# Berkeley-Speech-Group/sylber

Hardware: AMD Instinct MI355X
Metric: audio-sec/s encoded (sylber_base, 16 kHz, batched 10 s clips) (higher is better)
Workload: dtype bf16; 1 GPU; Segmenter forward (conv frontend + HuBERT-9L encoder + boundary detection + segment mean-pool), batch 32 x 10 s 16 kHz random waveforms per GPU, random-init sylber_base weights (BASELINE.json configs[1]); global_batch=32, frames_per_clip=499, parallelism=utterance-sharded x1, shards resident per rank, no data-path collective, rccl_ranks=1

## Files before the change

### include/sylber_hip.h

```cpp
#ifndef SYLBER_HIP_H
#define SYLBER_HIP_H

#include <stdint.h>

#ifdef __cplusplus
extern "C" {
#endif

#define SYLBER_MAX_LAYERS 12
#define SYLBER_HIDDEN 768
#define SYLBER_CONV_DIM 512

typedef struct sylber_ctx* sylber_t;

enum { SYLBER_BF16 = 0, SYLBER_FP32 = 1, SYLBER_FP8 = 2, SYLBER_FP16 = 3, SYLBER_MIXED16 = 4, SYLBER_SPLIT16 = 5 };

typedef struct {
    const float* q_w; const float* q_b;
    const float* k_w; const float* k_b;
    const float* v_w; const float* v_b;
    const float* o_w; const float* o_b;
    const float* ln1_w; const float* ln1_b;
    const float* ff1_w; const float* ff1_b;
    const float* ff2_w; const float* ff2_b;
// ... 276 lines not shown
int sylber_condition_units(sylber_mlp_t m, const float* c1_dev, int32_t K1, const float* c2_dev, int32_t K2, const int32_t* units_dev,
                           const int32_t* spans_dev, const int32_t* nunits_dev, const int32_t* frames_dev, int32_t B, int32_t T, int32_t S,
                           float* cond_dev, float* workspace_dev, void* stream);
int64_t sylber_condition_packed_workspace_floats(sylber_mlp_t m, int32_t B, int32_t S);
int sylber_condition_packed(sylber_mlp_t m, const float* hidden_dev, const int32_t* offsets_host, const int32_t* frames_host, int32_t B,
                            const int64_t* seg_dev, const int32_t* nseg_dev, const float* feat_dev, int32_t K, int32_t S, float norm_thr,
                            float* avg_hidden_dev, float* cond_dev, float* workspace_dev, void* stream);
int sylber_condition_units_packed(sylber_mlp_t m, const float* c1_dev, int32_t K1, const float* c2_dev, int32_t K2, const int32_t* units_dev,
                                  const int32_t* spans_dev, const int32_t* nunits_dev, const int32_t* frames_host, int32_t B, int32_t S,
                                  float* cond_dev, float* workspace_dev, void* stream);
int sylber_expand_units(const float* feats_dev, const int32_t* durations_dev, int32_t B, int32_t S, int32_t D, int32_t T, float* out_dev,
                        int32_t* workspace_dev, void* stream);

enum { SYLBER_OPT_GEMM_TILE = 1, SYLBER_OPT_ATTN_QUERIES_PER_WAVE = 2, SYLBER_OPT_GEMM_PERSISTENT = 3, SYLBER_OPT_FUSE_OUTPROJ_LN = 4,
       SYLBER_OPT_CONV0_VALU = 5, SYLBER_OPT_RESLN_PREFETCH = 6, SYLBER_OPT_FP8_ATTENTION = 7, SYLBER_OPT_GEMM_TAIL = 8, SYLBER_OPT_SEGMENT = 9, SYLBER_OPT_FP16_AUDIT = 10, SYLBER_OPT_GEMM_H192 = 11, SYLBER_OPT_GEMM_MODEL = 12, SYLBER_OPT_GEMM_MFMA16 = 13,
       SYLBER_OPT_PER_UTTERANCE = 14 };
int sylber_set_option(sylber_t h, int32_t key, int32_t value);
int sylber_get_fp16_audit(sylber_t h, const char** names, uint32_t* saturated, float* max_abs, int32_t cap);

int sylber_condition_features(sylber_mlp_t m, const float* features_dev, int32_t rows, float* cond_dev, float* workspace_dev,
                              void* stream);

enum { SYLBER_TAP_CONV0 = -1, SYLBER_TAP_PROJ = -2, SYLBER_TAP_POSCONV = -3 };
enum { SYLBER_LTAP_QKV = 0, SYLBER_LTAP_CTX = 1, SYLBER_LTAP_ATTN_SUM = 2, SYLBER_LTAP_LN1 = 3, SYLBER_LTAP_FFN1 = 4, SYLBER_LTAP_FFN2_SUM = 5 };
#define SYLBER_TAP_LAYER(l, k) (-(8 * ((l) + 1) + (k)))
#define SYLBER_TAP_CONV(i) (-(1024 + (i)))
int sylber_set_stop_stage(sylber_t h, int32_t stage);
int sylber_set_profiling(sylber_t h, int32_t enable);
int sylber_get_profile(sylber_t h, const char** names, float* ms, int32_t cap);
int sylber_set_graph_mode(sylber_t h, int32_t enable);
int64_t sylber_workspace_bytes(sylber_t h);
// ... 53 lines not shown
```

### sylber_amd/_lib.py

```python
from __future__ import annotations

import ctypes
import os
from ctypes import POINTER, c_char_p, c_float, c_int, c_int32, c_int64, c_void_p

_HERE = os.path.dirname(os.path.abspath(__file__))
LIB_PATH = os.path.join(_HERE, "libsylber_hip.so")
_DEV_LIB = False
MAX_LAYERS = 12

c_float_p = POINTER(c_float)


class SylberLayerWeights(ctypes.Structure):
    _fields_ = [(n, c_float_p) for n in (
        "q_w", "q_b", "k_w", "k_b", "v_w", "v_b", "o_w", "o_b", "ln1_w", "ln1_b",
        "ff1_w", "ff1_b", "ff2_w", "ff2_b", "ln2_w", "ln2_b")]


class SylberMlpHidden(ctypes.Structure):
    _fields_ = [(n, c_float_p) for n in ("lin_w", "lin_b", "ff1_w", "ff1_b", "ff2_w", "ff2_b", "ln_w", "ln_b")]


class SylberMlpWeights(ctypes.Structure):
# ... 220 lines not shown
    "sylber_cfm_tap_floats_packed": (c_int64, [c_void_p, c_int32, POINTER(c_int32), c_int32]),
    "sylber_debug_segment_scalars": (c_int, [c_void_p, c_void_p, c_int64, c_void_p, c_void_p, c_void_p, c_void_p, c_void_p, c_void_p, c_int64,
                                             c_void_p, c_void_p]),
}
CFM_TAP_CONDX, CFM_TAP_GB, CFM_TAP_XE, CFM_TAP_X0 = 1, 2, 3, 4
(CFM_BTAP_H_ATTN, CFM_BTAP_QKV, CFM_BTAP_Q, CFM_BTAP_K, CFM_BTAP_VT, CFM_BTAP_QKVF, CFM_BTAP_CTX, CFM_BTAP_X_ATTN, CFM_BTAP_H_FF, CFM_BTAP_FF,
 CFM_BTAP_G, CFM_BTAP_X_FF) = range(12)


def CFM_TAP(block: int, k: int) -> int:
    return 16 * (int(block) + 1) + int(k)
OPT_GEMM_TILE, OPT_ATTN_QUERIES_PER_WAVE, OPT_GEMM_PERSISTENT = 1, 2, 3
OPT_FUSE_OUTPROJ_LN, OPT_CONV0_VALU = 4, 5
OPT_FP8_ATTENTION, OPT_SEGMENT, OPT_PER_UTTERANCE = 7, 9, 14
OPT_GEMM_MODEL, OPT_GEMM_MFMA16 = 12, 13
TAP_CONV0, TAP_PROJ, TAP_POSCONV = -1, -2, -3
LTAP_QKV, LTAP_CTX, LTAP_ATTN_SUM, LTAP_LN1, LTAP_FFN1, LTAP_FFN2_SUM = 0, 1, 2, 3, 4, 5
LTAP_WIDTH = {LTAP_QKV: 2304, LTAP_CTX: 768, LTAP_ATTN_SUM: 768, LTAP_LN1: 768, LTAP_FFN1: 3072, LTAP_FFN2_SUM: 768}


def ltap_width(k: int, precision: str = "bf16", fp8_attention: bool = True) -> int:
    w = LTAP_WIDTH.get(int(k), 768)
    if precision != "fp8" or k in (LTAP_ATTN_SUM, LTAP_FFN2_SUM) or (k == LTAP_QKV and not fp8_attention):
        return w
    return 2 * w


def TAP_LAYER(l: int, k: int) -> int:
    return -(8 * (int(l) + 1) + int(k))

# ... 41 lines not shown
```

### sylber_amd/csrc/api.hip

```cpp
#include "ctx.h"

static thread_local char g_err[512] = "";
void syl_set_error(const char* what, const char* detail) { snprintf(g_err, sizeof(g_err), "%s: %s", what, detail); }
extern "C" const char* sylber_last_error(void) { return g_err; }

struct Packer {
    std::vector<char> host;
    size_t add(size_t bytes) { size_t off = (host.size() + 255) & ~(size_t)255; host.resize(off + bytes); return off; }
    size_t add_f32(const float* src, size_t n) { size_t o = add(n * 4); memcpy(host.data() + o, src, n * 4); return o; }
    int fmt = FMT_BF16;
    size_t add_bf16(const float* src, size_t n) {
        if (fmt == FMT_SPLIT) {
            size_t o = add(n * 4);
            bf16_t* d = (bf16_t*)(host.data() + o);
            for (size_t i = 0; i < n; ++i) { d[i] = f2h_host(src[i]); d[n + i] = f2h_host(src[i] - h2f_host(d[i])); }
            return o;
        }
        size_t o = add(n * 2);
        bf16_t* d = (bf16_t*)(host.data() + o);
        if (fmt == FMT_F16) for (size_t i = 0; i < n; ++i) d[i] = f2h_host(src[i]);
        else for (size_t i = 0; i < n; ++i) d[i] = f2bf(src[i]);
        return o;
    }
};
// ... 39 lines not shown
            for (int n = 0; n < 48; ++n)
                for (int cc = 0; cc < 48; ++cc)
                    for (int t = 0; t < 128; ++t)
                        tmp[(((size_t)g * 128 + t) * 64 + n) * 56 + cc] = w->pos_w[(((size_t)g * 48 + n) * 48 + cc) * 128 + t];
        if (!f32) o_posw = P.add_bf16(tmp.data(), tmp.size());
        else {
            std::vector<float> t32((size_t)16 * 128 * 64 * 52, 0.f);
            for (int g = 0; g < 16; ++g)
                for (int n = 0; n < 48; ++n)
                    for (int cc = 0; cc < 48; ++cc)
                        for (int t = 0; t < 128; ++t)
                            t32[(((size_t)g * 128 + t) * 64 + n) * 52 + cc] = w->pos_w[(((size_t)g * 48 + n) * 48 + cc) * 128 + t];
            o_posw = P.add_f32(t32.data(), t32.size());
        }
    }
    size_t o_posb = P.add_f32(w->pos_b, 768);
    size_t o_elw = P.add_f32(w->enc_ln_w, 768), o_elb = P.add_f32(w->enc_ln_b, 768);
    struct LOff { size_t wqkv, bqkv, wo, bo, l1w, l1b, w1, b1, w2, b2, l2w, l2b; } lo[SYLBER_MAX_LAYERS];
    for (int l = 0; l < w->num_layers; ++l) {
        const SylberLayerWeights& lw = w->layers[l];
        std::vector<float> qkv((size_t)2304 * 768), bq(2304);
        memcpy(qkv.data(), lw.q_w, 768 * 768 * 4);
        memcpy(qkv.data() + 768 * 768, lw.k_w, 768 * 768 * 4);
        memcpy(qkv.data() + 2 * 768 * 768, lw.v_w, 768 * 768 * 4);
        memcpy(bq.data(), lw.q_b, 768 * 4); memcpy(bq.data() + 768, lw.k_b, 768 * 4); memcpy(bq.data() + 1536, lw.v_b, 768 * 4);
        lo[l].wqkv = f32 ? P.add_f32(qkv.data(), qkv.size()) : P.add_bf16(qkv.data(), qkv.size()); lo[l].bqkv = P.add_f32(bq.data(), 2304);
        lo[l].wo = f32 ? P.add_f32(lw.o_w, 768 * 768) : P.add_bf16(lw.o_w, 768 * 768); lo[l].bo = P.add_f32(lw.o_b, 768);
        lo[l].l1w = P.add_f32(lw.ln1_w, 768); lo[l].l1b = P.add_f32(lw.ln1_b, 768);
        lo[l].w1 = f32 ? P.add_f32(lw.ff1_w, (size_t)3072 * 768) : P.add_bf16(lw.ff1_w, (size_t)3072 * 768); lo[l].b1 = P.add_f32(lw.ff1_b, 3072);
        lo[l].w2 = f32 ? P.add_f32(lw.ff2_w, (size_t)768 * 3072) : P.add_bf16(lw.ff2_w, (size_t)768 * 3072); lo[l].b2 = P.add_f32(lw.ff2_b, 768);
        lo[l].l2w = P.add_f32(lw.ln2_w, 768); lo[l].l2b = P.add_f32(lw.ln2_b, 768);
    }
    c->wbytes = P.host.size();
    if (hipMalloc((void**)&c->wbase, c->wbytes) != hipSuccess) { delete c; syl_set_error("sylber_create", "hipMalloc(weights) failed"); return 1; }
    if (hipMemcpy(c->wbase, P.host.data(), c->wbytes, hipMemcpyHostToDevice) != hipSuccess) {
        hipFree(c->wbase); delete c; syl_set_error("sylber_create", "weight upload failed"); return 1;
    }
    char* b = c->wbase;
    c->conv0_w = (float*)(b + o_conv0); c->gn_w = (float*)(b + o_gnw); c->gn_b = (float*)(b + o_gnb);
    c->conv_w[0] = nullptr;
    for (int i = 1; i < 7; ++i) { c->conv_w[i] = (bf16_t*)(b + o_conv[i]); c->conv_w32[i] = (float*)(b + o_conv[i]); }
    c->fp_w32 = (float*)(b + o_fpw); c->pos_w32 = (float*)(b + o_posw);
    c->fp_ln_w = (float*)(b + o_fplw); c->fp_ln_b = (float*)(b + o_fplb);
    c->fp_w = (bf16_t*)(b + o_fpw); c->fp_b = (float*)(b + o_fpb);
    c->pos_w = (bf16_t*)(b + o_posw); c->pos_b = (float*)(b + o_posb);
    c->enc_ln_w = (float*)(b + o_elw); c->enc_ln_b = (float*)(b + o_elb);
    for (int l = 0; l < w->num_layers; ++l) {
        LayerDev& d = c->L[l];
        d.wqkv = (bf16_t*)(b + lo[l].wqkv); d.bqkv = (float*)(b + lo[l].bqkv);
        d.wo = (bf16_t*)(b + lo[l].wo); d.bo = (float*)(b + lo[l].bo);
        d.ln1w = (float*)(b + lo[l].l1w); d.ln1b = (float*)(b + lo[l].l1b);
        d.w1 = (bf16_t*)(b + lo[l].w1); d.b1 = (float*)(b + lo[l].b1);
        d.w2 = (bf16_t*)(b + lo[l].w2); d.b2 = (float*)(b + lo[l].b2);
        d.ln2w = (float*)(b + lo[l].l2w); d.ln2b = (float*)(b + lo[l].l2b);
        c->L32[l].wqkv = (float*)(b + lo[l].wqkv); c->L32[l].wo = (float*)(b + lo[l].wo);
        c->L32[l].w1 = (float*)(b + lo[l].w1); c->L32[l].w2 = (float*)(b + lo[l].w2);
    }
    if (precision == SYLBER_FP8) {
        const size_t per_layer = (size_t)3072 * 768 + (size_t)3072 * 24 + (size_t)768 * 3072 + (size_t)768 * 96 +
                                 (size_t)2304 * 768 + (size_t)2304 * 24 + (size_t)768 * 768 + (size_t)768 * 24;
// ... 78 lines not shown
            GUARD_DEVICE(c->device);
            c->opt_audit16 = value > 0 ? 1 : 0;
            if (c->opt_audit16) {
                if (!c->audit_dev) HIP_TRY(hipMalloc((void**)&c->audit_dev, AUDIT_STAGES * 2 * sizeof(unsigned)));
                HIP_TRY(hipDeviceSynchronize());
                HIP_TRY(hipMemset(c->audit_dev, 0, AUDIT_STAGES * 2 * sizeof(unsigned)));
            }
            break;
        }
        case SYLBER_OPT_SEGMENT: c->opt_segment = value < 0 ? -1 : 0; break;
        case SYLBER_OPT_GEMM_MODEL: c->opt_gemm_model = value == 5 ? 5 : (value == 2 ? 2 : (value == 6 ? 6 : 0)); break;
        case SYLBER_OPT_GEMM_H192: c->opt_gemm_h192 = value < 0 ? -1 : 0; break;
        case SYLBER_OPT_GEMM_MFMA16: c->opt_gemm_mfma16 = value < 0 ? -1 : 0; break;
        case SYLBER_OPT_GEMM_TAIL: c->opt_gemm_tail = value < 0 ? -1 : (value > 0 ? value + 1 : 0); break;
        case SYLBER_OPT_PER_UTTERANCE: c->opt_per_utt = value == 1 ? 1 : 0; break;
        default: syl_set_error("sylber_set_option", "unknown option key"); return 1;
    }
    if (c->graph_mode) graphs_clear(c);
    return 0;
}
extern "C" int sylber_set_profiling(sylber_t c, int32_t enable) {
    if (!c) return 1;
    const char* nm[1]; float ms[1];
    sylber_get_profile(c, nm, ms, 0);
    c->prof_names.clear(); c->prof_ms.clear();
    c->profiling = enable;
    return 0;
}
extern "C" int64_t sylber_workspace_bytes(sylber_t c) { return c ? (int64_t)(c->ws_bytes + c->seg_scratch_floats * 4 + c->wbytes + c->f8bytes) : 0; }

// ... 96 lines not shown
```

### sylber_amd/csrc/ctx.h

```cpp
#pragma once
#include <stdio.h>
#include <stdlib.h>
#include <string.h>

#include <string>
#include <vector>

#include "../../include/sylber_hip.h"
#include "../../include/sylber_hip_dev.h"
#include "kernels.h"

struct DeviceGuard {
    int prev = -1; bool ok = true;
    explicit DeviceGuard(int dev) {
        if (hipGetDevice(&prev) != hipSuccess) prev = -1;
        if (prev != dev) ok = hipSetDevice(dev) == hipSuccess;
    }
    ~DeviceGuard() { int cur = -1; if (prev >= 0 && hipGetDevice(&cur) == hipSuccess && cur != prev) (void)hipSetDevice(prev); }
};
#define GUARD_DEVICE(dev)                                                                             \
    DeviceGuard _dg(dev);                                                                             \
    if (!_dg.ok) { syl_set_error("hipSetDevice", "cannot select the handle's device"); return 1; }

static const int CK[7] = {10, 3, 3, 3, 3, 2, 2};
// ... 9 lines not shown

struct ProfEntry { std::string name; hipEvent_t e0, e1; };
struct GraphEntry { int B, Lmax, stop_stage; const void* in; void* out; hipGraphExec_t exec; unsigned long long stamp; };

enum { AUD_CONV0 = 0, AUD_CONV6 = 6, AUD_LN512 = 7, AUD_XPAD = 8, AUD_LN = 9, AUD_Q = 10, AUD_K = 11, AUD_V = 12, AUD_CTX = 13, AUD_FFN1 = 14, AUDIT_STAGES = 15 };

struct sylber_ctx {
    int device = 0, precision = 0, num_layers = 9;
    int fmt = FMT_BF16;
    int fmt_conv = FMT_BF16;
    char* wbase = nullptr; size_t wbytes = 0;
    char* f8base = nullptr; size_t f8bytes = 0;
    float *conv0_w, *gn_w, *gn_b, *fp_ln_w, *fp_ln_b, *fp_b, *pos_b, *enc_ln_w, *enc_ln_b;
    bf16_t* conv_w[7];
    bf16_t *fp_w, *pos_w;
    LayerDev L[SYLBER_MAX_LAYERS];
    float* conv_w32[7]; float *fp_w32, *pos_w32;
    struct { float *wqkv, *wo, *w1, *w2; } L32[SYLBER_MAX_LAYERS];
    char* ws = nullptr; size_t ws_bytes = 0;
    int ws_B = 0, ws_Lmax = 0;
    float* seg_scratch = nullptr; size_t seg_scratch_floats = 0;
    int stop_stage = 0;
    const float* dbg_ss = nullptr; int dbg_ss_B = 0;
    int opt_gemm_cfg = 0, opt_attn_qw = 0, opt_gemm_persist = 0;
    int opt_fuse_ln = 0;
    int opt_conv0_valu = 0;
    int opt_audit16 = 0;
    unsigned* audit_dev = nullptr;
    int opt_segment = 0;
    int opt_gemm_model = 0;
    int opt_gemm_mfma16 = 0;
    int opt_gemm_h192 = 0;
    int opt_gemm_tail = 0;
    int opt_attn8 = 0;
    int opt_resln_pre = 0;
    int opt_per_utt = 0;
    bool graph_mode = false;
    std::vector<GraphEntry> graphs; unsigned long long graph_clock = 0;
    int profiling = 0;
    std::vector<ProfEntry> prof;
    std::vector<hipEvent_t> ev_pool;
    std::vector<std::string> prof_names; std::vector<float> prof_ms;
};

void graphs_clear(sylber_ctx* c);

struct ProfScope {
    sylber_ctx* c; hipStream_t s; bool on;
    ProfScope(sylber_ctx* c_, hipStream_t s_, const char* name) : c(c_), s(s_), on(c_->profiling != 0) {
        if (!on) return;
// ... 14 lines not shown
```

### sylber_amd/csrc/forward.hip

```cpp
#include "ctx.h"

extern "C" int32_t sylber_num_frames(int32_t n) {
    for (int i = 0; i < 7; ++i) n = (n - CK[i]) / CS[i] + 1;
    return n;
}

static int frames_needed(int Lmax) {
    int n = Lmax, tp = 0;
    for (int i = 0; i < 7; ++i) {
        n = (n - CK[i]) / CS[i] + 1;
        const int f = 1 << (6 - i);
        const int need = (n + f - 1) / f;
        tp = need > tp ? need : tp;
    }
    return tp;
}
static int padded_frames(int Lmax) { return (frames_needed(Lmax) + 31) & ~31; }
extern "C" int32_t sylber_padded_frames(int32_t n_samples) { return n_samples < 400 ? 0 : padded_frames(n_samples); }

#define SYL_SLOT_ALIGN 64
extern "C" int sylber_packed_layout(const int32_t* samples_host, int32_t B, int32_t* offsets, int32_t* frames) {
    if (!samples_host || !offsets || !frames || B < 1) { syl_set_error("sylber_packed_layout", "need B >= 1 and non-null arrays"); return 1; }
    const long long cap = (long long)INT32_MAX / SYL_SLOT_SAMPLES;
    long long off = 0;
// ... 337 lines not shown
        LnArgs a = {};
        a.in = feats; a.in_bf16 = 1; a.ld_in = 512; a.gamma = c->fp_ln_w; a.beta = c->fp_ln_b;
        a.out_bf16 = w.ln512; a.ld_bf16 = 512; a.M = M; a.D = 512; a.fmt = c->fmt; a.fmt_in = c->fmt_conv;
        a.in_lo = feats_lo; a.out_lo = p.lo_ln512;
        RUN("ln512", launch_layernorm(a, s));
        GemmArgs g = linear(w.ln512, p.lo_ln512, c->fp_w, c->fp_b, 768, 512);
        g.out0 = w.xf32; g.ld0 = 768; g.out1 = w.xpad; g.Tp = p.Tp; g.T = p.T; g.valid = w.valid; g.xpad_rows = p.Tp + 128; g.out_lo = p.lo_xpad;
        RUN("gemm_proj", launch_gemm_bf16(EPI_PROJ, g, s));
        if (pk) RUN("zero_slot_tails", launch_zero_slot_tails(w.xf32, w.xpad, pk->slot, pk->frames, pk->nclip, pk->tail_max, s));
        AUDIT(aud_e, AUD_LN512, w.ln512, M, 512, 512);
        AUDIT(aud_e, AUD_XPAD, w.xpad, (long)B * (p.Tp + 128), 768, 768);
        return 0;
    }

    int posconv() {
        if (pk) RUN("posconv", launch_posconv_packed(w.xpad, c->pos_w, c->pos_b, w.xf32, w.pre, pk->nclip, pk->slot_max, pk->slot, pk->frames, s, c->fmt));
        else RUN("posconv", launch_posconv(w.xpad, c->pos_w, c->pos_b, w.xf32, w.pre, B, p.Tp, split ? 2 : 1, s, c->fmt, p.lo_xpad, (long)16 * 128 * 64 * 56));
        return 0;
    }

    int layernorm(const float* gam, const float* bet, bool last) {
        LnArgs a = {};
        a.in = w.pre; a.in_bf16 = 0; a.ld_in = 768; a.gamma = gam; a.beta = bet; a.M = M; a.D = 768; a.fmt = c->fmt; a.fmt_in = c->fmt;
        if (last) { a.out_f32 = hidden_dev; a.ld_f32 = 768; a.Tp = p.Tp; a.T = p.T; }
        else if (f8) { a.out_fp8 = w8.h; a.ld_fp8 = 768; a.out_scale = w8.hs; a.scale_rows = w8.Mp; a.out_stats = w.stats; }
        else { a.out_bf16 = w.h; a.ld_bf16 = 768; a.out_stats = w.stats; a.out_lo = p.lo_hbf; }
        if (launch_layernorm(a, s)) return 1;
        AUDIT(aud_e && !last && !f8, AUD_LN, w.h, M, 768, 768);
        return 0;
    }

    int tap_rows16(const bf16_t* buf, long lo, int W) {
// ... 298 lines not shown
    const bool f32 = c->precision == SYLBER_FP32;
    const Plan p = f32 ? make_plan_f32(B, Lmax) : make_plan(B, Lmax, c->precision == SYLBER_SPLIT16 ? 2 : 1);
    if (begin_call(c, p, {{p.o_valid, valid.data(), B}, {p.o_rows, c->opt_per_utt ? rows0.data() : nullptr, B}}, s)) return 1;
    c->dbg_ss = (const float*)(c->ws + p.o_ss); c->dbg_ss_B = B;
    if (f32) return ForwardF32(c, p, wav_dev, hidden_dev, s).run();
    if (!c->graph_mode || c->profiling || c->opt_audit16 || s == nullptr || c->stop_stage < 0) return Forward(c, p, wav_dev, hidden_dev, s, nullptr).run();
    return forward_graph(c, p, wav_dev, hidden_dev, s);
}

extern "C" int sylber_forward_packed(sylber_t c, const float* wav_dev, const int32_t* samples_host, int32_t B, float* hidden_dev, void* stream) {
    if (!c || !wav_dev || !samples_host || !hidden_dev) { syl_set_error("sylber_forward_packed", "null argument"); return 1; }
    if (c->precision != SYLBER_BF16 && c->precision != SYLBER_FP16) {
        syl_set_error("sylber_forward_packed", "packed batches run in the bf16 and fp16 precisions only"); return 1;
    }
    if (c->graph_mode) { syl_set_error("sylber_forward_packed", "not available in graph mode (sylber_set_graph_mode)"); return 1; }
    if (c->stop_stage != 0 || c->opt_conv0_valu != 0 || c->opt_attn_qw != 0) {
        syl_set_error("sylber_forward_packed", "not available with a stop stage, SYLBER_OPT_CONV0_VALU or SYLBER_OPT_ATTN_QUERIES_PER_WAVE"); return 1;
    }
    std::vector<int32_t> off(B > 0 ? B + 1 : 1), fr(B > 0 ? B : 1);
    if (sylber_packed_layout(samples_host, B, off.data(), fr.data())) return 1;
    const int Ptot = off[B];
    std::vector<int32_t> tab(3 * (size_t)B + 2), rows0(B);
    int slot_max = 0, tail_max = 0, nmax = 0;
    tab[2 * B + 1] = 0;
    for (int b = 0; b < B; ++b) {
        const int sl = off[b + 1] - off[b];
        slot_max = sl > slot_max ? sl : slot_max;
        tail_max = sl - fr[b] > tail_max ? sl - fr[b] : tail_max;
        rows0[b] = (samples_host[b] - CK[0]) / CS[0] + 1;
        nmax = samples_host[b] > nmax ? samples_host[b] : nmax;
        tab[B + 1 + b] = fr[b];
        tab[2 * B + 2 + b] = tab[2 * B + 1 + b] + (fr[b] + 127) / 128;
// ... 44 lines not shown
```

### sylber_amd/csrc/kernels.h

```cpp
#pragma once
#include "common.h"

enum GemmAct { ACT_NONE = 0, ACT_GELU_FAST = 1, ACT_GELU_ERF = 2, ACT_GELU_ERF7 = 3 };
enum GemmEpi {
    EPI_BF16 = 0,
    EPI_F32 = 1,
    EPI_F32_RES = 2,
    EPI_QK = 3,
    EPI_PROJ = 4,
    EPI_MXFP8 = 7,
    EPI_QK8 = 8,
    EPI_F32_RESLN = 6,
};

struct GemmArgs {
    const bf16_t* X; long ldx;
    const bf16_t* W;
    int M, N, K;
    int M_store;
    const float* bias;
    int act;
    void* out0; long ld0;
    void* out1; void* out2;
    const float* res; long ldres;
// ... 59 lines not shown
};
int launch_gemm_f32(const GemmArgsF32& a, hipStream_t s);
int launch_km_normalize(const float* x, float* y, int n, int D, hipStream_t s);
int launch_km_sqnorm(const float* c, float* out, int K, int D, hipStream_t s);

int launch_conv0_stats(const float* wav, int B, int Lmax, int L0, double* partials, int nchunk, hipStream_t s, const int* rows = nullptr,
                       const int* slot = nullptr);
int launch_conv0_finalize(const double* partials, int nchunk, const float* w0, const float* gn_w, const float* gn_b,
                          int B, int L0, float* scale_shift, hipStream_t s, const int* rows = nullptr);
int launch_conv0_gn_gelu(const float* wav, int B, int Lmax, int L0, int R0, const float* w0,
                         const float* scale_shift, void* out, int out_f32, hipStream_t s, int fmt = 0, long out_lo = 0, int valu16 = 0);
int launch_conv0_packed(const float* wav, int B, int total_samples, int slot_max, const int* rows, const int* slot, const float* w0,
                        const float* scale_shift, bf16_t* out, int fmt, hipStream_t s);
int launch_zero_slot_tails(float* x, bf16_t* xpad, const int* slot, const int* frames, int B, int tail_max, hipStream_t s);
int launch_posconv_packed(const bf16_t* xpad, const bf16_t* wpk, const float* bias, const float* x_f32, float* out, int B, int slot_max,
                          const int* slot, const int* frames, hipStream_t s, int fmt);
int launch_attention_packed(const bf16_t* q, const bf16_t* k, const bf16_t* vt, const int* pk, int nclip, int total_qb, bf16_t* ctx,
                            int Ptot, hipStream_t s, int fmt);

struct LnArgs {
    const void* in; int in_bf16; long ld_in;
    int fmt;
    int fmt_in;
    const float* res; long ld_res;
    const float* gamma; const float* beta;
    float* out_f32; long ld_f32;
    bf16_t* out_bf16; long ld_bf16;
    uint8_t* out_fp8; long ld_fp8;
    uint8_t* out_scale; long scale_rows;
    float* out_stats;
    int M, D;
    int Tp, T;
    long in_lo, out_lo;
};
int launch_layernorm(const LnArgs& a, hipStream_t s);

int launch_attention(const bf16_t* q, const bf16_t* k, const bf16_t* vt, const int* valid, bf16_t* ctx, int B, int T,
                     int Tp, int Tpv, int qw, hipStream_t s, int fmt = 0, long lo_qk = 0, long lo_vt = 0, long lo_ctx = 0);
int launch_attention_f8(const uint8_t* q8, const uint8_t* qs, const uint8_t* k8, const uint8_t* ks, const uint8_t* v8, const uint8_t* vs,
                        const int* valid, void* ctx, uint8_t* ctx_scale, long scale_rows, int B, int T, int Tp, int Tpv, hipStream_t s);
int launch_attention_f8out(const bf16_t* q, const bf16_t* k, const bf16_t* vt, const int* valid, uint8_t* ctx8, uint8_t* ctx_scale,
                           long scale_rows, int B, int T, int Tp, int Tpv, int qw, hipStream_t s);
int launch_attention_f32(const float* q, const float* k, const float* v, const int* valid, float* ctx, int B, int T,
                         int Tp, hipStream_t s);

int launch_posconv(const bf16_t* xpad, const bf16_t* wpk, const float* bias, const float* x_f32, float* out, int B,
                   int Tp, int act, hipStream_t s, int fmt = 0, long x_lo = 0, long w_lo = 0);
int launch_posconv_f32(const float* xpad, const float* w, const float* bias, const float* x_f32, float* out, int B,
                       int Tp, hipStream_t s);

int launch_segment(const float* hidden, int B, int T, int D, float norm_thr, float merge_thr, int64_t* seg, int* nseg,
                   float* feat, float* scratch, hipStream_t s, int mode = 0, const int* frames = nullptr, const int* row0 = nullptr);
size_t segment_scratch_floats(int B, int T, int D);

int launch_upload_ints(int* dst, const int32_t* vals_host, int n, int add, hipStream_t s);
int launch_f32_to_bf16(const float* in, bf16_t* out, size_t n, hipStream_t s);
int launch_f32_to_split16(const float* in, bf16_t* out, long lo_off, size_t n, hipStream_t s);
int launch_bf16_to_f32_rows(const bf16_t* in, long ld_in, float* out, int B, int Tp, int T, int D, hipStream_t s, int fmt = 0, long in_lo = 0);
enum { MXTAP_ROWS = 0, MXTAP_HEADS = 1, MXTAP_VT = 2 };
int launch_mxfp8_to_f32_rows(const uint8_t* data, const uint8_t* scale, int layout, long pitch, float* out, long ld_out, int val_col, int exp_col,
                             int B, int Tp, int T, int W, hipStream_t s);
int launch_tap_qkv(const bf16_t* q, const bf16_t* k, const bf16_t* vt, float* out, int B, int T, int Tp, int Tpv, hipStream_t s, int fmt, long lo_qk, long lo_vt);
// ... 1 lines not shown
```

### sylber_amd/csrc/posconv.hip

```cpp
#include "kernels.h"
#include "lds_dma.h"

#define PC_BM 256
#define PC_XROW 112
#define PC_XWIN (384 * PC_XROW)
#define PC_SLAB (64 * 112)
#define PC_TAPS_PER_STEP 2
#define PC_STEP (PC_TAPS_PER_STEP * PC_SLAB)
#define PC_LDS (PC_XWIN + 2 * PC_STEP)

template <int ACT, int FMT>
__global__ __launch_bounds__(512, 4) void posconv_bf16_kernel(const bf16_t* __restrict__ xpad, const bf16_t* __restrict__ wpk,
                                                              const float* __restrict__ bias, const float* __restrict__ x_f32,
                                                              float* __restrict__ out, int Tp, long x_lo, long w_lo,
                                                              const int* __restrict__ slot, const int* __restrict__ frames) {
    extern __shared__ __attribute__((aligned(256))) char smem[];
    char* xwin = smem;
    char* wring = smem + PC_XWIN;
    const int tid = threadIdx.x, wave = tid >> 6, lane = tid & 63;
    const int ql = lane & 31, h = lane >> 5;
    const int t0 = blockIdx.x * PC_BM, g = blockIdx.y, b = blockIdx.z;
    const int rows_per_b = Tp + 128;
    int s0 = 0, Tb = 0, Tpb = Tp;
    if (slot) {
// ... 74 lines not shown
                const int nl = 32 * nf + 8 * gg + 4 * h;
                if (nl >= SYL_POSC) continue;
                const int n = g * SYL_POSC + nl;
                const float4 bb = *(const float4*)(bias + n);
                const float4 rr = *(const float4*)(x_f32 + m * SYL_HIDDEN + n);
                float v0 = acc[nf][4 * gg + 0] + bb.x, v1 = acc[nf][4 * gg + 1] + bb.y;
                float v2 = acc[nf][4 * gg + 2] + bb.z, v3 = acc[nf][4 * gg + 3] + bb.w;
                if constexpr (ACT == 2 && FMT == FMT_SPLIT) { v0 = gelu_erf7(v0); v1 = gelu_erf7(v1); v2 = gelu_erf7(v2); v3 = gelu_erf7(v3); }
                else if constexpr (ACT == 2) { v0 = gelu_erf(v0); v1 = gelu_erf(v1); v2 = gelu_erf(v2); v3 = gelu_erf(v3); }
                else { v0 = gelu_fast(v0); v1 = gelu_fast(v1); v2 = gelu_fast(v2); v3 = gelu_fast(v3); }
                *(float4*)(out + m * SYL_HIDDEN + n) = make_float4(rr.x + v0, rr.y + v1, rr.z + v2, rr.w + v3);
            }
    }
}

static int posconv_attrs() {
    static PerDeviceOnce attr_once;
    if (attr_once.need()) {
        HIP_TRY(hipFuncSetAttribute((const void*)posconv_bf16_kernel<1, FMT_BF16>, hipFuncAttributeMaxDynamicSharedMemorySize, PC_LDS));
        HIP_TRY(hipFuncSetAttribute((const void*)posconv_bf16_kernel<2, FMT_BF16>, hipFuncAttributeMaxDynamicSharedMemorySize, PC_LDS));
        HIP_TRY(hipFuncSetAttribute((const void*)posconv_bf16_kernel<1, FMT_F16>, hipFuncAttributeMaxDynamicSharedMemorySize, PC_LDS));
        HIP_TRY(hipFuncSetAttribute((const void*)posconv_bf16_kernel<2, FMT_SPLIT>, hipFuncAttributeMaxDynamicSharedMemorySize, PC_LDS));
    }
    return 0;
}

int launch_posconv(const bf16_t* xpad, const bf16_t* wpk, const float* bias, const float* x_f32, float* out, int B, int Tp,
                   int act, hipStream_t s, int fmt, long x_lo, long w_lo) {
    dim3 grid((Tp + PC_BM - 1) / PC_BM, SYL_POSG, B);
    if (posconv_attrs()) return 1;
    if (fmt == FMT_SPLIT) {
        hipLaunchKernelGGL((posconv_bf16_kernel<2, FMT_SPLIT>), grid, dim3(512), PC_LDS, s, xpad, wpk, bias, x_f32, out, Tp, x_lo, w_lo, nullptr, nullptr);
        HIP_TRY(hipGetLastError());
        return 0;
    }
    if (fmt == FMT_F16 && act == 2) { syl_set_error("launch_posconv", "the erf GELU (act 2) has no fp16 instantiation"); return 1; }
    if (fmt == FMT_F16) hipLaunchKernelGGL((posconv_bf16_kernel<1, FMT_F16>), grid, dim3(512), PC_LDS, s, xpad, wpk, bias, x_f32, out, Tp, 0L, 0L, nullptr, nullptr);
    else if (act == 2) hipLaunchKernelGGL((posconv_bf16_kernel<2, FMT_BF16>), grid, dim3(512), PC_LDS, s, xpad, wpk, bias, x_f32, out, Tp, 0L, 0L, nullptr, nullptr);
    else hipLaunchKernelGGL((posconv_bf16_kernel<1, FMT_BF16>), grid, dim3(512), PC_LDS, s, xpad, wpk, bias, x_f32, out, Tp, 0L, 0L, nullptr, nullptr);
    HIP_TRY(hipGetLastError());
    return 0;
}

int launch_posconv_packed(const bf16_t* xpad, const bf16_t* wpk, const float* bias, const float* x_f32, float* out, int B, int slot_max,
                          const int* slot, const int* frames, hipStream_t s, int fmt) {
    if (fmt != FMT_BF16 && fmt != FMT_F16) { syl_set_error("launch_posconv_packed", "bf16 / fp16 only"); return 1; }
    if (posconv_attrs()) return 1;
    dim3 grid((slot_max + PC_BM - 1) / PC_BM, SYL_POSG, B);
    if (fmt == FMT_F16) hipLaunchKernelGGL((posconv_bf16_kernel<1, FMT_F16>), grid, dim3(512), PC_LDS, s, xpad, wpk, bias, x_f32, out, 0, 0L, 0L, slot, frames);
    else hipLaunchKernelGGL((posconv_bf16_kernel<1, FMT_BF16>), grid, dim3(512), PC_LDS, s, xpad, wpk, bias, x_f32, out, 0, 0L, 0L, slot, frames);
    HIP_TRY(hipGetLastError());
    return 0;
}
```

### sylber_amd/segmenter.py

```python
from __future__ import annotations

import ctypes
import math
import os
import collections
import threading
import time
import weakref
from pathlib import Path
from typing import Dict, List, Optional, Sequence, Union

import numpy as np
import torch

from . import _lib
from .ingest import ingest_file
from .weights import (NUM_LAYERS, expected_shapes, fold_pos_conv_weight, normalize_keys, synthetic_state_dict)

FRAME_RATE = 50
SLOT_SAMPLES = 320
PACKED_PRECISIONS = ("bf16", "fp16")


def _ptr(t: torch.Tensor):
# ... 322 lines not shown
    def set_graph_mode(self, enable: bool = True) -> None:
        _lib.check(self.lib.sylber_set_graph_mode(self.handle, 1 if enable else 0), "sylber_set_graph_mode")
        self._graph_stream = torch.cuda.Stream(device=self.device) if enable else None

    def _check_packed(self, what: str) -> None:
        if self.precision not in PACKED_PRECISIONS:
            raise ValueError("%s: packed batches run in precision %s only (this encoder: %r)" % (what, " / ".join(map(repr, PACKED_PRECISIONS)),
                                                                                                   self.precision))
        if getattr(self, "_graph_stream", None) is not None:
            raise ValueError("%s: packed batches do not run in graph mode (set_graph_mode(False))" % what)
        if self._opts.get(_lib.OPT_SEGMENT, 0) < 0:
            raise ValueError("%s: packed boundary detection needs the wide segmenter (SYLBER_OPT_SEGMENT = 0, not -1)" % what)
        if (self._opts.get(_lib.OPT_ATTN_QUERIES_PER_WAVE, 0) in (32, 64) or self._opts.get(_lib.OPT_CONV0_VALU, 0) > 0):
            raise ValueError("%s: packed batches need SYLBER_OPT_ATTN_QUERIES_PER_WAVE and SYLBER_OPT_CONV0_VALU at their defaults" % what)

    def forward_packed_raw(self, wav: torch.Tensor, lengths: Sequence[int], out: Optional[torch.Tensor] = None, layout=None) -> torch.Tensor:
        self._check_packed("forward_packed")
        n = [int(x) for x in lengths]
        offsets, _ = packed_layout(n) if layout is None else layout
        P = int(offsets[-1])
        assert wav.is_cuda and wav.dtype == torch.float32 and wav.is_contiguous() and wav.numel() == SLOT_SAMPLES * P
        if out is None:
            out = torch.empty(P, 768, dtype=torch.float32, device=wav.device)
        assert out.is_contiguous() and out.numel() >= P * 768
        with torch.cuda.device(wav.device):
            st = self.lib.sylber_forward_packed(self.handle, ctypes.c_void_p(wav.data_ptr()), (ctypes.c_int32 * len(n))(*n), len(n),
                                                ctypes.c_void_p(out.data_ptr()), _stream_ptr(wav.device))
        _lib.check(st, "sylber_forward_packed")
        return out

    def forward_packed(self, wavs: Sequence[torch.Tensor]):
        self._check_packed("forward_packed")
        rows = [torch.as_tensor(w).reshape(-1) for w in wavs]
        lengths = [int(r.numel()) for r in rows]
        offsets, frames = packed_layout(lengths)
        wav = torch.zeros(SLOT_SAMPLES * int(offsets[-1]), dtype=torch.float32, device=self.device)
        for i, r in enumerate(rows):
            a = SLOT_SAMPLES * int(offsets[i])
            wav[a:a + lengths[i]] = r.to(self.device, torch.float32)
        return self.forward_packed_raw(wav, lengths), offsets, frames

    def segment_packed(self, hidden: torch.Tensor, lengths: Sequence[int], norm_threshold: float, merge_threshold: float,
                       with_features: bool = True, out=None, layout=None):
        self._check_packed("segment_packed")
        n = [int(x) for x in lengths]
        offsets, frames = packed_layout(n) if layout is None else layout
        assert hidden.is_cuda and hidden.dtype == torch.float32 and hidden.is_contiguous() and hidden.numel() >= int(offsets[-1]) * 768
        B, K, D = len(n), int(frames.max()), 768
        if out is not None:
            seg, nseg, feats = out
        else:
            seg = torch.empty(B, K, 2, dtype=torch.int64, device=hidden.device)
            nseg = torch.empty(B, dtype=torch.int32, device=hidden.device)
            feats = torch.empty(B, K, D, dtype=torch.float32, device=hidden.device) if with_features else None
        with torch.cuda.device(hidden.device):
# ... 555 lines not shown
```

Baseline: 67520 audio-sec/s.

## Add 16x16x32 MFMA positional-conv kernel with prepacked weights and LDS ring

Adds a new grouped positional-convolution kernel built on 16x16x32 bf16/fp16 MFMA instructions. It uses a host-repacked weight layout that pairs taps, stages the input window in LDS, and streams weights through a 2- or 3-slot LDS ring filled by async global-to-LDS loads. Bias, GELU and the residual add are fused into its epilogue. The kernel is selected by a new option whose default value routes both the padded and packed paths to it. The change also allows a posconv stop stage for packed batches, and it adds an extra weight copy in device memory.

```diff
diff --git a/include/sylber_hip.h b/include/sylber_hip.h
--- a/include/sylber_hip.h
+++ b/include/sylber_hip.h
@@ -314,7 +314,7 @@
 
 enum { SYLBER_OPT_GEMM_TILE = 1, SYLBER_OPT_ATTN_QUERIES_PER_WAVE = 2, SYLBER_OPT_GEMM_PERSISTENT = 3, SYLBER_OPT_FUSE_OUTPROJ_LN = 4,
        SYLBER_OPT_CONV0_VALU = 5, SYLBER_OPT_RESLN_PREFETCH = 6, SYLBER_OPT_FP8_ATTENTION = 7, SYLBER_OPT_GEMM_TAIL = 8, SYLBER_OPT_SEGMENT = 9, SYLBER_OPT_FP16_AUDIT = 10, SYLBER_OPT_GEMM_H192 = 11, SYLBER_OPT_GEMM_MODEL = 12, SYLBER_OPT_GEMM_MFMA16 = 13,
-       SYLBER_OPT_PER_UTTERANCE = 14 };
+       SYLBER_OPT_PER_UTTERANCE = 14, SYLBER_OPT_POSCONV = 15 };
 int sylber_set_option(sylber_t h, int32_t key, int32_t value);
 int sylber_get_fp16_audit(sylber_t h, const char** names, uint32_t* saturated, float* max_abs, int32_t cap);
 
diff --git a/sylber_amd/_lib.py b/sylber_amd/_lib.py
--- a/sylber_amd/_lib.py
+++ b/sylber_amd/_lib.py
@@ -258,6 +258,7 @@
 OPT_FUSE_OUTPROJ_LN, OPT_CONV0_VALU = 4, 5
 OPT_FP8_ATTENTION, OPT_SEGMENT, OPT_PER_UTTERANCE = 7, 9, 14
 OPT_GEMM_MODEL, OPT_GEMM_MFMA16 = 12, 13
+OPT_POSCONV = 15
 TAP_CONV0, TAP_PROJ, TAP_POSCONV = -1, -2, -3
 LTAP_QKV, LTAP_CTX, LTAP_ATTN_SUM, LTAP_LN1, LTAP_FFN1, LTAP_FFN2_SUM = 0, 1, 2, 3, 4, 5
 LTAP_WIDTH = {LTAP_QKV: 2304, LTAP_CTX: 768, LTAP_ATTN_SUM: 768, LTAP_LN1: 768, LTAP_FFN1: 3072, LTAP_FFN2_SUM: 768}
diff --git a/sylber_amd/csrc/api.hip b/sylber_amd/csrc/api.hip
--- a/sylber_amd/csrc/api.hip
+++ b/sylber_amd/csrc/api.hip
@@ -77,6 +77,17 @@
             o_posw = P.add_f32(t32.data(), t32.size());
         }
     }
+    size_t o_posw16 = 0;
+    const bool pos16 = !f32 && c->fmt != FMT_SPLIT;
+    if (pos16) {
+        std::vector<float> tmp((size_t)16 * 64 * 48 * 96);
+        for (int g = 0; g < 16; ++g)
+            for (int n = 0; n < 48; ++n)
+                for (int cc = 0; cc < 48; ++cc)
+                    for (int t = 0; t < 128; ++t)
+                        tmp[(((size_t)g * 64 + t / 2) * 48 + n) * 96 + (t & 1) * 48 + cc] = w->pos_w[(((size_t)g * 48 + n) * 48 + cc) * 128 + t];
+        o_posw16 = P.add_bf16(tmp.data(), tmp.size());
+    }
     size_t o_posb = P.add_f32(w->pos_b, 768);
     size_t o_elw = P.add_f32(w->enc_ln_w, 768), o_elb = P.add_f32(w->enc_ln_b, 768);
     struct LOff { size_t wqkv, bqkv, wo, bo, l1w, l1b, w1, b1, w2, b2, l2w, l2b; } lo[SYLBER_MAX_LAYERS];
@@ -107,6 +118,7 @@
     c->fp_ln_w = (float*)(b + o_fplw); c->fp_ln_b = (float*)(b + o_fplb);
     c->fp_w = (bf16_t*)(b + o_fpw); c->fp_b = (float*)(b + o_fpb);
     c->pos_w = (bf16_t*)(b + o_posw); c->pos_b = (float*)(b + o_posb);
+    c->pos_w16 = pos16 ? (bf16_t*)(b + o_posw16) : nullptr;
     c->enc_ln_w = (float*)(b + o_elw); c->enc_ln_b = (float*)(b + o_elb);
     for (int l = 0; l < w->num_layers; ++l) {
         LayerDev& d = c->L[l];
@@ -215,6 +227,7 @@
         case SYLBER_OPT_GEMM_MFMA16: c->opt_gemm_mfma16 = value < 0 ? -1 : 0; break;
         case SYLBER_OPT_GEMM_TAIL: c->opt_gemm_tail = value < 0 ? -1 : (value > 0 ? value + 1 : 0); break;
         case SYLBER_OPT_PER_UTTERANCE: c->opt_per_utt = value == 1 ? 1 : 0; break;
+        case SYLBER_OPT_POSCONV: c->opt_posconv = value < 0 ? -1 : (value <= 2 ? value : 0); break;
         default: syl_set_error("sylber_set_option", "unknown option key"); return 1;
     }
     if (c->graph_mode) graphs_clear(c);
diff --git a/sylber_amd/csrc/ctx.h b/sylber_amd/csrc/ctx.h
--- a/sylber_amd/csrc/ctx.h
+++ b/sylber_amd/csrc/ctx.h
@@ -47,6 +47,7 @@
     float *conv0_w, *gn_w, *gn_b, *fp_ln_w, *fp_ln_b, *fp_b, *pos_b, *enc_ln_w, *enc_ln_b;
     bf16_t* conv_w[7];
     bf16_t *fp_w, *pos_w;
+    bf16_t* pos_w16 = nullptr;
     LayerDev L[SYLBER_MAX_LAYERS];
     float* conv_w32[7]; float *fp_w32, *pos_w32;
     struct { float *wqkv, *wo, *w1, *w2; } L32[SYLBER_MAX_LAYERS];
@@ -67,6 +68,7 @@
     int opt_gemm_tail = 0;
     int opt_attn8 = 0;
     int opt_resln_pre = 0;
+    int opt_posconv = 0;
     int opt_per_utt = 0;
     bool graph_mode = false;
     std::vector<GraphEntry> graphs; unsigned long long graph_clock = 0;
diff --git a/sylber_amd/csrc/forward.hip b/sylber_amd/csrc/forward.hip
--- a/sylber_amd/csrc/forward.hip
+++ b/sylber_amd/csrc/forward.hip
@@ -375,8 +375,8 @@
     }
 
     int posconv() {
-        if (pk) RUN("posconv", launch_posconv_packed(w.xpad, c->pos_w, c->pos_b, w.xf32, w.pre, pk->nclip, pk->slot_max, pk->slot, pk->frames, s, c->fmt));
-        else RUN("posconv", launch_posconv(w.xpad, c->pos_w, c->pos_b, w.xf32, w.pre, B, p.Tp, split ? 2 : 1, s, c->fmt, p.lo_xpad, (long)16 * 128 * 64 * 56));
+        if (pk) RUN("posconv", launch_posconv_packed(w.xpad, c->pos_w, c->pos_b, w.xf32, w.pre, pk->nclip, pk->slot_max, pk->slot, pk->frames, s, c->fmt, c->pos_w16, c->opt_posconv));
+        else RUN("posconv", launch_posconv(w.xpad, c->pos_w, c->pos_b, w.xf32, w.pre, B, p.Tp, split ? 2 : 1, s, c->fmt, p.lo_xpad, (long)16 * 128 * 64 * 56, c->pos_w16, c->opt_posconv));
         return 0;
     }
 
@@ -705,8 +705,8 @@
         syl_set_error("sylber_forward_packed", "packed batches run in the bf16 and fp16 precisions only"); return 1;
     }
     if (c->graph_mode) { syl_set_error("sylber_forward_packed", "not available in graph mode (sylber_set_graph_mode)"); return 1; }
-    if (c->stop_stage != 0 || c->opt_conv0_valu != 0 || c->opt_attn_qw != 0) {
-        syl_set_error("sylber_forward_packed", "not available with a stop stage, SYLBER_OPT_CONV0_VALU or SYLBER_OPT_ATTN_QUERIES_PER_WAVE"); return 1;
+    if ((c->stop_stage != 0 && c->stop_stage != SYLBER_TAP_POSCONV) || c->opt_conv0_valu != 0 || c->opt_attn_qw != 0) {
+        syl_set_error("sylber_forward_packed", "not available with a stop stage other than SYLBER_TAP_POSCONV, SYLBER_OPT_CONV0_VALU or SYLBER_OPT_ATTN_QUERIES_PER_WAVE"); return 1;
     }
     std::vector<int32_t> off(B > 0 ? B + 1 : 1), fr(B > 0 ? B : 1);
     if (sylber_packed_layout(samples_host, B, off.data(), fr.data())) return 1;
diff --git a/sylber_amd/csrc/kernels.h b/sylber_amd/csrc/kernels.h
--- a/sylber_amd/csrc/kernels.h
+++ b/sylber_amd/csrc/kernels.h
@@ -97,7 +97,7 @@
                         const float* scale_shift, bf16_t* out, int fmt, hipStream_t s);
 int launch_zero_slot_tails(float* x, bf16_t* xpad, const int* slot, const int* frames, int B, int tail_max, hipStream_t s);
 int launch_posconv_packed(const bf16_t* xpad, const bf16_t* wpk, const float* bias, const float* x_f32, float* out, int B, int slot_max,
-                          const int* slot, const int* frames, hipStream_t s, int fmt);
+                          const int* slot, const int* frames, hipStream_t s, int fmt, const bf16_t* w16 = nullptr, int variant = -1);
 int launch_attention_packed(const bf16_t* q, const bf16_t* k, const bf16_t* vt, const int* pk, int nclip, int total_qb, bf16_t* ctx,
                             int Ptot, hipStream_t s, int fmt);
 
@@ -128,7 +128,7 @@
                          int Tp, hipStream_t s);
 
 int launch_posconv(const bf16_t* xpad, const bf16_t* wpk, const float* bias, const float* x_f32, float* out, int B,
-                   int Tp, int act, hipStream_t s, int fmt = 0, long x_lo = 0, long w_lo = 0);
+                   int Tp, int act, hipStream_t s, int fmt = 0, long x_lo = 0, long w_lo = 0, const bf16_t* w16 = nullptr, int variant = -1);
 int launch_posconv_f32(const float* xpad, const float* w, const float* bias, const float* x_f32, float* out, int B,
                        int Tp, hipStream_t s);
 
diff --git a/sylber_amd/csrc/posconv.hip b/sylber_amd/csrc/posconv.hip
--- a/sylber_amd/csrc/posconv.hip
+++ b/sylber_amd/csrc/posconv.hip
@@ -112,9 +112,157 @@
     }
 }
 
+#define P16_BM 256
+#define P16_XROW 96
+#define P16_XWIN (384 * P16_XROW)
+#define P16_WROW 224
+#define P16_GSTEP (SYL_POSC * 96 * 2)
+#define P16_PIECES 11
+#define P16_SLOT (P16_PIECES * 1024)
+#define P16_LDS(NS) (P16_XWIN + (NS) * P16_SLOT)
+
+template <int FMT> struct Mfma16 {
+    static __device__ __forceinline__ f32x4_t mfma(bf16x8_t a, bf16x8_t b, f32x4_t c) { return __builtin_amdgcn_mfma_f32_16x16x32_bf16(a, b, c, 0, 0, 0); }
+};
+template <> struct Mfma16<FMT_F16> {
+    static __device__ __forceinline__ f32x4_t mfma(bf16x8_t a, bf16x8_t b, f32x4_t c) {
+        return __builtin_amdgcn_mfma_f32_16x16x32_f16(__builtin_bit_cast(f16x8_t, a), __builtin_bit_cast(f16x8_t, b), c, 0, 0, 0);
+    }
+};
+
+template <int FMT, int NS>
+__global__ __launch_bounds__(256, 2) void posconv16_kernel(const bf16_t* __restrict__ xpad, const bf16_t* __restrict__ w16,
+                                                           const float* __restrict__ bias, const float* __restrict__ x_f32,
+                                                           float* __restrict__ out, int Tp, const int* __restrict__ slot,
+                                                           const int* __restrict__ frames) {
+    extern __shared__ __attribute__((aligned(256))) char smem[];
+    char* xwin = smem;
+    char* wring = smem + P16_XWIN;
+    const int tid = threadIdx.x, wave = __builtin_amdgcn_readfirstlane(tid >> 6), lane = tid & 63;
+    const int fr = lane & 15, kq = lane >> 4;
+    const int t0 = blockIdx.x * P16_BM, g = blockIdx.y, b = blockIdx.z;
+    const int rows_per_b = Tp + 128;
+    int s0 = 0, Tb = 0, Tpb = Tp;
+    if (slot) {
+        s0 = slot[b]; Tb = frames[b]; Tpb = slot[b + 1] - s0;
+        if (t0 >= Tpb) return;
+    }
+
+    {
+        const bf16_t* xb = xpad + (slot ? (size_t)s0 : (size_t)b * rows_per_b) * SYL_HIDDEN + g * SYL_POSC;
+        uint4 v[9];
+#pragma unroll
+        for (int i = 0; i < 9; ++i) {
+            const int idx = tid + 256 * i;
+            const int r = idx / 6, ch = idx - r * 6;
+            if (slot) {
+                const int f = t0 + r - 64;
+                v[i] = (f >= 0 && f < Tb) ? *(const uint4*)(xb + (size_t)(f + 64) * SYL_HIDDEN + ch * 8) : make_uint4(0u, 0u, 0u, 0u);
+            } else {
+                int row = t0 + r; row = row < rows_per_b ? row : rows_per_b - 1;
+                v[i] = *(const uint4*)(xb + (size_t)row * SYL_HIDDEN + ch * 8);
+            }
+        }
+#pragma unroll
+        for (int i = 0; i < 9; ++i) *(uint4*)(xwin + (tid + 256 * i) * 16) = v[i];
+    }
+    const __amdgpu_buffer_rsrc_t rwg = make_rsrc((const char*)w16 + (size_t)g * (SYL_POSK / 2) * P16_GSTEP);
+    int voff[3];
+#pragma unroll
+    for (int i = 0; i < 3; ++i) {
+        const int ci = (wave + 4 * i) * 64 + lane;
+        int row = ci / 14, cc = ci - row * 14;
+        row = row < SYL_POSC ? row : SYL_POSC - 1; cc = cc < 12 ? cc : 11;
+        voff[i] = row * 192 + cc * 16;
+    }
+    auto stage = [&](int step, int buf) {
+        char* dst = wring + buf * P16_SLOT;
+#pragma unroll
+        for (int i = 0; i < 3; ++i) {
+            const int piece = wave + 4 * i;
+            if (piece < P16_PIECES) glds16b(rwg, voff[i], step * P16_GSTEP, dst + piece * 1024);
+        }
+    };
+
+    f32x4_t acc[4][3];
+#pragma unroll
+    for (int fb = 0; fb < 4; ++fb)
+#pragma unroll
+        for (int nb = 0; nb < 3; ++nb) acc[fb][nb] = f32x4_t{0.f, 0.f, 0.f, 0.f};
+
+    const int xfrag = (wave * 64 + fr) * P16_XROW + kq * 16;
+    const int wfrag = fr * P16_WROW + kq * 16;
+    constexpr int nsteps = SYL_POSK / 2;
+#pragma unroll
+    for (int i = 0; i < NS - 1; ++i) stage(i, i);
+    bf16x8_t wf[2][3], xf[2][4];
+    auto load_w = [&](bf16x8_t (&d)[3], const char* p) {
+#pragma unroll
+        for (int nb = 0; nb < 3; ++nb) d[nb] = *(const bf16x8_t*)(p + nb * 16 * P16_WROW);
+    };
+    auto load_x = [&](bf16x8_t (&d)[4], const char* p) {
+#pragma unroll
+        for (int fb = 0; fb < 4; ++fb) d[fb] = *(const bf16x8_t*)(p + fb * 16 * P16_XROW);
+    };
+    static_assert(nsteps % 2 == 0, "two steps per trip");
+#pragma unroll 1
+    for (int st2 = 0; st2 < nsteps; st2 += 2) {
+#pragma unroll
+        for (int hh = 0; hh < 2; ++hh) {
+            const int st = st2 + hh;
+            if (NS == 3 && st + 1 < nsteps) {
+                if (wave == 3) wait_vmcnt<2>(); else wait_vmcnt<3>();
+            } else wait_vmcnt<0>();
+            __syncthreads();
+            if (st + NS - 1 < nsteps) stage(st + NS - 1, (st + NS - 1) % NS);
+            const char* wb = wring + (st % NS) * P16_SLOT + wfrag;
+            const char* xs = xwin + xfrag + st * (2 * P16_XROW);
+            if (st == 0) load_x(xf[0], xs);
+            load_w(wf[hh], wb);
+#pragma unroll
+            for (int sl = 0; sl < 3; ++sl) {
+                const int cur = (3 * hh + sl) & 1, nxt = cur ^ 1;
+                if (sl < 2) { load_w(wf[nxt], wb + (sl + 1) * 64); load_x(xf[nxt], xs + (sl + 1) * 64); }
+                else if (st + 1 < nsteps) load_x(xf[nxt], xs + 2 * P16_XROW);
+#pragma unroll
+                for (int fb = 0; fb < 4; ++fb)
+#pragma unroll
+                    for (int nb = 0; nb < 3; ++nb) acc[fb][nb] = Mfma16<FMT>::mfma(wf[cur][nb], xf[cur][fb], acc[fb][nb]);
+            }
+        }
+    }
+#pragma unroll
+    for (int fb = 0; fb < 4; ++fb) {
+        const int t = t0 + wave * 64 + fb * 16 + fr;
+        if (t >= Tpb) continue;
+        const size_t m = slot ? (size_t)s0 + t : (size_t)b * Tp + t;
+#pragma unroll
+        for (int nb = 0; nb < 3; ++nb) {
+            const int n = g * SYL_POSC + nb * 16 + kq * 4;
+            const float4 bb = *(const float4*)(bias + n);
+            const float4 rr = *(const float4*)(x_f32 + m * SYL_HIDDEN + n);
+            const float v0 = gelu_fast(acc[fb][nb][0] + bb.x), v1 = gelu_fast(acc[fb][nb][1] + bb.y);
+            const float v2 = gelu_fast(acc[fb][nb][2] + bb.z), v3 = gelu_fast(acc[fb][nb][3] + bb.w);
+            *(float4*)(out + m * SYL_HIDDEN + n) = make_float4(rr.x + v0, rr.y + v1, rr.z + v2, rr.w + v3);
+        }
+    }
+}
+
+#define P16_LDS_ONE_PER_CU (96 * 1024)
+template <int FMT>
+static void posconv16_launch(int variant, dim3 grid, hipStream_t s, const bf16_t* xpad, const bf16_t* w16, const float* bias, const float* x_f32,
+                             float* out, int Tp, const int* slot, const int* frames) {
+    if (variant == 1) hipLaunchKernelGGL((posconv16_kernel<FMT, 3>), grid, dim3(256), P16_LDS(3), s, xpad, w16, bias, x_f32, out, Tp, slot, frames);
+    else hipLaunchKernelGGL((posconv16_kernel<FMT, 2>), grid, dim3(256), variant == 2 ? P16_LDS_ONE_PER_CU : P16_LDS(2), s, xpad, w16, bias, x_f32, out, Tp, slot, frames);
+}
+
 static int posconv_attrs() {
     static PerDeviceOnce attr_once;
     if (attr_once.need()) {
+        HIP_TRY(hipFuncSetAttribute((const void*)posconv16_kernel<FMT_BF16, 2>, hipFuncAttributeMaxDynamicSharedMemorySize, P16_LDS_ONE_PER_CU));
+        HIP_TRY(hipFuncSetAttribute((const void*)posconv16_kernel<FMT_F16, 2>, hipFuncAttributeMaxDynamicSharedMemorySize, P16_LDS_ONE_PER_CU));
+        HIP_TRY(hipFuncSetAttribute((const void*)posconv16_kernel<FMT_BF16, 3>, hipFuncAttributeMaxDynamicSharedMemorySize, P16_LDS(3)));
+        HIP_TRY(hipFuncSetAttribute((const void*)posconv16_kernel<FMT_F16, 3>, hipFuncAttributeMaxDynamicSharedMemorySize, P16_LDS(3)));
         HIP_TRY(hipFuncSetAttribute((const void*)posconv_bf16_kernel<1, FMT_BF16>, hipFuncAttributeMaxDynamicSharedMemorySize, PC_LDS));
         HIP_TRY(hipFuncSetAttribute((const void*)posconv_bf16_kernel<2, FMT_BF16>, hipFuncAttributeMaxDynamicSharedMemorySize, PC_LDS));
         HIP_TRY(hipFuncSetAttribute((const void*)posconv_bf16_kernel<1, FMT_F16>, hipFuncAttributeMaxDynamicSharedMemorySize, PC_LDS));
@@ -124,9 +272,16 @@
 }
 
 int launch_posconv(const bf16_t* xpad, const bf16_t* wpk, const float* bias, const float* x_f32, float* out, int B, int Tp,
-                   int act, hipStream_t s, int fmt, long x_lo, long w_lo) {
+                   int act, hipStream_t s, int fmt, long x_lo, long w_lo, const bf16_t* w16, int variant) {
     dim3 grid((Tp + PC_BM - 1) / PC_BM, SYL_POSG, B);
     if (posconv_attrs()) return 1;
+    if (variant >= 0 && act == 1 && (fmt == FMT_BF16 || fmt == FMT_F16)) {
+        if (!w16) { syl_set_error("launch_posconv", "the 16x16x32 kernel needs its weight pack"); return 1; }
+        if (fmt == FMT_F16) posconv16_launch<FMT_F16>(variant, grid, s, xpad, w16, bias, x_f32, out, Tp, nullptr, nullptr);
+        else posconv16_launch<FMT_BF16>(variant, grid, s, xpad, w16, bias, x_f32, out, Tp, nullptr, nullptr);
+        HIP_TRY(hipGetLastError());
+        return 0;
+    }
     if (fmt == FMT_SPLIT) {
         hipLaunchKernelGGL((posconv_bf16_kernel<2, FMT_SPLIT>), grid, dim3(512), PC_LDS, s, xpad, wpk, bias, x_f32, out, Tp, x_lo, w_lo, nullptr, nullptr);
         HIP_TRY(hipGetLastError());
@@ -141,10 +296,17 @@
 }
 
 int launch_posconv_packed(const bf16_t* xpad, const bf16_t* wpk, const float* bias, const float* x_f32, float* out, int B, int slot_max,
-                          const int* slot, const int* frames, hipStream_t s, int fmt) {
+                          const int* slot, const int* frames, hipStream_t s, int fmt, const bf16_t* w16, int variant) {
     if (fmt != FMT_BF16 && fmt != FMT_F16) { syl_set_error("launch_posconv_packed", "bf16 / fp16 only"); return 1; }
     if (posconv_attrs()) return 1;
     dim3 grid((slot_max + PC_BM - 1) / PC_BM, SYL_POSG, B);
+    if (variant >= 0) {
+        if (!w16) { syl_set_error("launch_posconv_packed", "the 16x16x32 kernel needs its weight pack"); return 1; }
+        if (fmt == FMT_F16) posconv16_launch<FMT_F16>(variant, grid, s, xpad, w16, bias, x_f32, out, 0, slot, frames);
+        else posconv16_launch<FMT_BF16>(variant, grid, s, xpad, w16, bias, x_f32, out, 0, slot, frames);
+        HIP_TRY(hipGetLastError());
+        return 0;
+    }
     if (fmt == FMT_F16) hipLaunchKernelGGL((posconv_bf16_kernel<1, FMT_F16>), grid, dim3(512), PC_LDS, s, xpad, wpk, bias, x_f32, out, 0, 0L, 0L, slot, frames);
     else hipLaunchKernelGGL((posconv_bf16_kernel<1, FMT_BF16>), grid, dim3(512), PC_LDS, s, xpad, wpk, bias, x_f32, out, 0, 0L, 0L, slot, frames);
     HIP_TRY(hipGetLastError());
diff --git a/sylber_amd/segmenter.py b/sylber_amd/segmenter.py
--- a/sylber_amd/segmenter.py
+++ b/sylber_amd/segmenter.py
@@ -360,7 +360,8 @@
         if (self._opts.get(_lib.OPT_ATTN_QUERIES_PER_WAVE, 0) in (32, 64) or self._opts.get(_lib.OPT_CONV0_VALU, 0) > 0):
             raise ValueError("%s: packed batches need SYLBER_OPT_ATTN_QUERIES_PER_WAVE and SYLBER_OPT_CONV0_VALU at their defaults" % what)
 
-    def forward_packed_raw(self, wav: torch.Tensor, lengths: Sequence[int], out: Optional[torch.Tensor] = None, layout=None) -> torch.Tensor:
+    def forward_packed_raw(self, wav: torch.Tensor, lengths: Sequence[int], out: Optional[torch.Tensor] = None, layout=None,
+                           stop_stage: int = 0) -> torch.Tensor:
         self._check_packed("forward_packed")
         n = [int(x) for x in lengths]
         offsets, _ = packed_layout(n) if layout is None else layout
@@ -369,13 +370,19 @@
         if out is None:
             out = torch.empty(P, 768, dtype=torch.float32, device=wav.device)
         assert out.is_contiguous() and out.numel() >= P * 768
-        with torch.cuda.device(wav.device):
-            st = self.lib.sylber_forward_packed(self.handle, ctypes.c_void_p(wav.data_ptr()), (ctypes.c_int32 * len(n))(*n), len(n),
-                                                ctypes.c_void_p(out.data_ptr()), _stream_ptr(wav.device))
+        if stop_stage:
+            _lib.check(self.lib.sylber_set_stop_stage(self.handle, int(stop_stage)), "sylber_set_stop_stage")
+        try:
+            with torch.cuda.device(wav.device):
+                st = self.lib.sylber_forward_packed(self.handle, ctypes.c_void_p(wav.data_ptr()), (ctypes.c_int32 * len(n))(*n), len(n),
+                                                    ctypes.c_void_p(out.data_ptr()), _stream_ptr(wav.device))
+        finally:
+            if stop_stage:
+                self.lib.sylber_set_stop_stage(self.handle, 0)
         _lib.check(st, "sylber_forward_packed")
         return out
 
-    def forward_packed(self, wavs: Sequence[torch.Tensor]):
+    def forward_packed(self, wavs: Sequence[torch.Tensor], stop_stage: int = 0):
         self._check_packed("forward_packed")
         rows = [torch.as_tensor(w).reshape(-1) for w in wavs]
         lengths = [int(r.numel()) for r in rows]
@@ -384,7 +391,7 @@
         for i, r in enumerate(rows):
             a = SLOT_SAMPLES * int(offsets[i])
             wav[a:a + lengths[i]] = r.to(self.device, torch.float32)
-        return self.forward_packed_raw(wav, lengths), offsets, frames
+        return self.forward_packed_raw(wav, lengths, stop_stage=stop_stage), offsets, frames
 
     def segment_packed(self, hidden: torch.Tensor, lengths: Sequence[int], norm_threshold: float, merge_threshold: float,
                        with_features: bool = True, out=None, layout=None):
```

After: 67900 audio-sec/s (median of 6 runs). No clear change (+0.6%).
